# genetics-statistics/GEMMA

Measured on AMD Instinct MI355X. Metric: SNPs/s (-lmm 1 Wald) at n=20k on 1/2/4/8 MI355X; U^T x HBM GB/s vs roofline, higher is better.
Workload: dtype f64 (U^T x as int8-digit MFMA products with exact int32 accumulation; every column of U scaled by its exact maximum and rounded to 6 base-256 digits = 2^-48 of that maximum -- fp64 keeps 2^-53 per entry; value_strict / strict_leg (7g6m: U^T x at or below the fp64 GEMM's own error) and fp64_gemm_path

## Files before the change

gemma_amd/build.py:

```python
import os
import shutil
import subprocess

HERE = os.path.dirname(os.path.abspath(__file__))
CSRC = os.path.join(HERE, "csrc")
LIB = os.path.join(HERE, "libgemma_hip.so")
UNITS = {
    "gemma_hip.hip": ["dgemm_mfma.hip.h", "lmm_grid.hip.h", "i8gemm.hip.h", "i8gemm_sparse.hip.h", "i8gemm_sparse2.hip.h", "i8gemm_sparse2_r16.hip.h", "i8gemm_dense16.hip.h", "lmm_assoc.hip.h",
                      "lmm_search.hip.h", "comm.hip.h", "comm_shm.hpp", "kin_i8.hip.h", "ingest.hip.h", "qc.hip.h", "lm_assoc.hip.h", "mvlmm.hip.h",
                      "mvlmm_kernels.hip.h", "eigh_tu.h", "tu_common.h",
                      "abi_kinship.inc.h", "abi_eigen_qc.inc.h", "abi_lmm_stage.inc.h", "abi_utx.inc.h", "abi_lmm_batch.inc.h",
                      "abi_mvlmm.inc.h", "abi_gxe_lm.inc.h", "abi_kept_comm.inc.h", "abi_vc.inc.h", "vc_tu.h", "abi_prdt.inc.h", "prdt_tu.h",
                      "abi_mqs.inc.h", "mqs_tu.h"],
    "eigh_tu.hip": ["dgemm_mfma.hip.h", "eigh.hip.h", "eigh2.hip.h", "eigh_tu.h", "tu_common.h"],
    "vc_tu.hip": ["dgemm_mfma.hip.h", "spd_inv.hip.h", "vc.hip.h", "vc_tu.h", "tu_common.h", "host_linalg.h", "../../include/gemma_vc_hybrid.hpp"],
    "prdt_tu.hip": ["dgemm_mfma.hip.h", "geno_mv.hip.h", "dev_common.hip.h", "eigh_tu.h", "prdt_tu.h", "tu_common.h"],
    "mqs_tu.hip": ["dgemm_mfma.hip.h", "mqs.hip.h", "dev_common.hip.h", "mqs_tu.h", "tu_common.h", "host_linalg.h"],
    "mvlmm_kernels.hip": ["mvlmm.hip.h", "mvlmm_kernels.hip.h"],
    "mvlmm_kernels_wide.hip": ["mvlmm.hip.h", "mvlmm_kernels.hip.h"],
    "mvlmm_kernels_rt.hip": ["mvlmm.hip.h", "mvlmm_kernels.hip.h"],
    "mvlmm_kernels_d6.hip": ["mvlmm.hip.h", "mvlmm_kernels.hip.h"],
    "mvlmm_kernels_d7.hip": ["mvlmm.hip.h", "mvlmm_kernels.hip.h"],
    "mvlmm_kernels_d8.hip": ["mvlmm.hip.h", "mvlmm_kernels.hip.h"],
}
PUBLIC_HEADER_USERS = ("gemma_hip.hip", "eigh_tu.hip", "vc_tu.hip", "prdt_tu.hip", "mqs_tu.hip")
SOURCES = list(UNITS)
HEADERS = sorted({h for hs in UNITS.values() for h in hs})


def hipcc():
    for cand in (os.environ.get("HIPCC"), "/opt/rocm/bin/hipcc", shutil.which("hipcc")):
        if cand and os.path.exists(cand):
            return cand
    raise RuntimeError("hipcc not found: the gfx950 library cannot be built")


def stale():
    if not os.path.exists(LIB):
        return True
    t = os.path.getmtime(LIB)
    deps = [os.path.join(CSRC, f) for f in SOURCES + HEADERS]
# ... 37 lines not shown
```

gemma_amd/csrc/abi_utx.inc.h:

```cpp

struct I8Dims {
  size_t n, ldk, npad, lpad, mrows;
  int fuse, digits, nplanes;
  int mdrop;
  int complete;
  int epi;
};
static const int *i8_anymiss(const I8Dims &d) { return d.complete ? g_ctx.i8_rowsur.as<int>() + d.lpad : nullptr; }
static int i8_sparse_mode() { return g_ctx.knobs.i8_sparse; }
static int i8_begin(size_t l, I8Dims *d, hipStream_t s, bool allow_epi = true) {
  int rc = i8_prepare_u(s);
  if (rc) return rc;
  d->n = g_ctx.cfg.n; d->ldk = g_ctx.i8_ldk; d->npad = g_ctx.i8_npad;
  d->lpad = round_up(l, i8_sparse_mode() == 2 ? (size_t)S2_BM : (size_t)I8P_BM); d->mrows = 2 * d->lpad;
  d->fuse = (g_ctx.knobs.i8_fuse && (double)d->n * 2.0 * 128.0 * 257.0 < 2147483648.0) ? 1 : 0;
  d->digits = g_ctx.i8_digits;
  d->nplanes = d->fuse ? (d->digits + 1) / 2 : d->digits;
  d->mdrop = (g_ctx.knobs.i8_mdrop && d->fuse && d->digits == 7 && i8_sparse_mode() == 2 && g_ctx.knobs.i8_rows == 16) ? 1 : 0;
  d->complete = (g_ctx.knobs.i8_complete && i8_sparse_mode() == 2 && g_ctx.knobs.i8_rows == 16) ? 1 : 0;
  d->epi = (allow_epi && g_ctx.knobs.i8_epilogue && i8_sparse_mode() == 2 && g_ctx.knobs.i8_rows == 16 && d->nplanes >= 2) ? 1 : 0;
  const size_t c_elems = (size_t)(d->nplanes - d->epi) * d->mrows * d->npad;
  if (g_ctx.i8_A.reserve(d->lpad * d->ldk) || g_ctx.i8_C.reserve(c_elems * 4) || g_ctx.i8_mean.reserve(l * 8))
    return fail(GEMMA_HIP_ENOMEM, "lmm_batch: int8 product buffers (%zu bytes)", d->lpad * d->ldk + c_elems * 4);
  if (d->lpad != l) HIPCHK(hipMemsetAsync(g_ctx.i8_A.p, 0, d->lpad * d->ldk, s));
  return GEMMA_HIP_OK;
}

static int i8_meta_build(const I8Dims &d, hipStream_t s) {
  const int mode = i8_sparse_mode();
  if (mode == 0) return GEMMA_HIP_OK;
  ProfScope ps(GEMMA_STAGE_INGEST, s);
  const size_t nk = d.ldk / I8_BK, total = d.lpad * nk * (mode == 2 ? 4 : 2);
  if (g_ctx.i8_meta.reserve(total * sizeof(uint4)) || g_ctx.i8_rowsur.reserve((d.lpad + 1) * sizeof(int)))
    return fail(GEMMA_HIP_ENOMEM, "lmm_batch: mask words of the sparse product");
  HIPCHK(hipMemsetAsync(g_ctx.i8_rowsur.p, 0, (d.lpad + 1) * sizeof(int), s));
  if (mode == 2)
    hipLaunchKernelGGL(sparse2_meta_kernel, dim3((unsigned)((total + 255) / 256)), dim3(256), 0, s, g_ctx.i8_A.as<int8_t>(),
                       (long)d.lpad, (long)d.ldk, g_ctx.i8_meta.as<uint4>(), g_ctx.i8_rowsur.as<int>(),
                       const_cast<int *>(i8_anymiss(d)));
  else
    hipLaunchKernelGGL(sparse_meta_kernel, dim3((unsigned)((total + 255) / 256)), dim3(256), 0, s, g_ctx.i8_A.as<int8_t>(),
                       (long)d.lpad, (long)d.ldk, g_ctx.i8_meta.as<uint4>(), g_ctx.i8_rowsur.as<int>());
  HIPCHK(hipGetLastError());
  g_ctx.i8_flag_at = (mode == 2 && d.complete) ? (long)d.lpad : -1;
  g_ctx.i8_rowsur_n = (long)d.lpad;
  return GEMMA_HIP_OK;
}

static int raster_for(int tiles_m, int tiles_n, int rb, hipStream_t s, const int2 **map_d) {
  Ctx::RasterSlot *lru = &g_ctx.i8_raster[0];
  for (auto &r : g_ctx.i8_raster) {
    if (r.tm == tiles_m && r.tn == tiles_n && r.rb == rb && r.dev.p) {
      r.used = ++g_ctx.i8_raster_clock;
      *map_d = r.dev.as<int2>();
      return GEMMA_HIP_OK;
    }
    if (r.used < lru->used) lru = &r;
// ... 21 lines not shown
  ProfScope ps(GEMMA_STAGE_UTX_GEMM, s);
  static bool attr_set = false;
  if (!attr_set) {
    HIPCHK(hipFuncSetAttribute(reinterpret_cast<const void *>(i8gemm_packed_kernel_t<true>),
                               hipFuncAttributeMaxDynamicSharedMemorySize, 3 * I8P_STAGE));
    attr_set = true;
  }
  I8PackArgs g;
  g.A = g_ctx.i8_A.as<int8_t>();
  g.Bt = g_ctx.i8_Bt.as<int8_t>();
  g.C = g_ctx.i8_C.as<int>();
  g.ldk = (long)d.ldk; g.ldc = (long)d.npad;
  g.strideB = (long)(d.npad * d.ldk); g.strideC = (long)(d.mrows * d.npad);
  g.m_row0 = (long)d.lpad;
  g.tiles_m = (int)(d.lpad / I8P_BM); g.tiles_n = (int)(d.npad / I8_BN);
  g.nk = (int)(d.ldk / I8_BK);
  g.gm = g_ctx.knobs.i8_gm;
  g.fuse = d.fuse;
  g.digits = d.digits;
  const dim3 grid((unsigned)(g.tiles_m * g.tiles_n), (unsigned)d.nplanes);
  if (mode == 2) {
    static bool attr3 = false;
    if (!attr3) {
      HIPCHK(hipFuncSetAttribute(reinterpret_cast<const void *>(i8gemm_sparse2_kernel),
                                 hipFuncAttributeMaxDynamicSharedMemorySize, S2_NST * S2_STAGE));
      HIPCHK(hipFuncSetAttribute(reinterpret_cast<const void *>(i8gemm_sparse2_r16_kernel),
                                 hipFuncAttributeMaxDynamicSharedMemorySize, S2_R16_LDS));
      HIPCHK(hipFuncSetAttribute(reinterpret_cast<const void *>(i8gemm_sparse2_r16_g_kernel),
                                 hipFuncAttributeMaxDynamicSharedMemorySize, S2_R16_LDS));
      HIPCHK(hipFuncSetAttribute(reinterpret_cast<const void *>(i8gemm_sparse2_r16_ep_kernel),
                                 hipFuncAttributeMaxDynamicSharedMemorySize, S2_R16_LDS));
      HIPCHK(hipFuncSetAttribute(reinterpret_cast<const void *>(i8gemm_sparse2_r16_ep_g_kernel),
                                 hipFuncAttributeMaxDynamicSharedMemorySize, S2_R16_LDS));
      attr3 = true;
    }
    Sparse2Args g2;
    g2.AM = g_ctx.i8_meta.as<uint4>() + (row0 / S2_BM) * (size_t)g.nk * S2_BM * 4;
    g2.Bt = g.Bt; g2.C = g.C + row0 * (size_t)g.ldc - (d.epi ? g.strideC : 0); g2.ldk = g.ldk; g2.ldc = g.ldc; g2.strideB = g.strideB; g2.strideC = g.strideC;
    g2.m_row0 = g.m_row0;
    g2.tiles_m = (int)(rows_pad / S2_BM); g2.tiles_n = (int)(d.npad / S2_BN);
    g2.nk = g.nk; g2.gm = g.gm; g2.fuse = g.fuse; g2.digits = g.digits;
    int raster_rb = 0;
    {
      const int rb = g_ctx.knobs.i8_raster;
      if (rb > 0) {
        const int2 *map_d = nullptr;
        int rc_map = raster_for(g2.tiles_m, g2.tiles_n, rb, s, &map_d);
        if (rc_map) return rc_map;
        g2.tile_map = map_d;
        raster_rb = rb;
      }
    }
    note_utx_kernel(g_ctx.knobs.i8_rows == 32 ? GEMMA_UTX_KERNEL_RECORDS_R32 : GEMMA_UTX_KERNEL_RECORDS_R16, d.digits, d.fuse,
                    raster_rb);
    if (g_ctx.knobs.i8_rows == 32) {
      hipLaunchKernelGGL(i8gemm_sparse2_kernel, dim3((unsigned)(g2.tiles_m * g2.tiles_n), (unsigned)d.nplanes), dim3(512),
                         S2_NST * S2_STAGE, s, g2);
    } else if (d.epi) {
      const unsigned wgs = (unsigned)(g2.tiles_m * g2.tiles_n);
      g2.anymiss = i8_anymiss(d);
      g2.plane0 = 1;
      g2.run_if = g2.anymiss ? 1 : 0;
      hipLaunchKernelGGL(i8gemm_sparse2_r16_kernel, dim3(wgs, (unsigned)d.nplanes - 1u), dim3(512), S2_R16_LDS, s, g2);
      if (g2.anymiss) {
        g2.run_if = 2;
        hipLaunchKernelGGL(i8gemm_sparse2_r16_g_kernel, dim3(wgs, (unsigned)d.nplanes - 1u), dim3(512), S2_R16_LDS, s, g2);
      }
      g2.plane0 = 0;
      g2.UtX = UtX + row0 * ldx; g2.ldx = (long)ldx; g2.l = (long)rows; g2.n = (long)d.n;
      g2.mean = g_ctx.i8_mean.as<double>() + row0; g2.qinv = g_ctx.i8_qinv.as<double>();
      g2.m_scale = 1.0; g2.nplanes = d.nplanes;
      if (d.mdrop) {
        g2.run_if = 0;
        hipLaunchKernelGGL(i8gemm_sparse2_r16_ep_g_kernel, dim3(wgs, 1u), dim3(512), S2_R16_LDS, s, g2);
      } else {
        g2.run_if = g2.anymiss ? 1 : 0;
        hipLaunchKernelGGL(i8gemm_sparse2_r16_ep_kernel, dim3(wgs, 1u), dim3(512), S2_R16_LDS, s, g2);
        if (g2.anymiss) {
          g2.run_if = 2;
          hipLaunchKernelGGL(i8gemm_sparse2_r16_ep_g_kernel, dim3(wgs, 1u), dim3(512), S2_R16_LDS, s, g2);
        }
      }
    } else {
      const unsigned wgs = (unsigned)(g2.tiles_m * g2.tiles_n), first = d.mdrop ? 1u : 0u;
      g2.anymiss = i8_anymiss(d);
      g2.plane0 = (int)first;
      g2.run_if = g2.anymiss ? 1 : 0;
      hipLaunchKernelGGL(i8gemm_sparse2_r16_kernel, dim3(wgs, (unsigned)d.nplanes - first), dim3(512), S2_R16_LDS, s, g2);
      if (g2.anymiss) {
        g2.run_if = 2;
        hipLaunchKernelGGL(i8gemm_sparse2_r16_g_kernel, dim3(wgs, (unsigned)d.nplanes - first), dim3(512), S2_R16_LDS, s, g2);
      }
      if (d.mdrop) {
        g2.plane0 = 0; g2.run_if = 0;
        hipLaunchKernelGGL(i8gemm_sparse2_r16_g_kernel, dim3(wgs, 1u), dim3(512), S2_R16_LDS, s, g2);
      }
    }
  } else if (sparse) {
    static bool attr2 = false;
    if (!attr2) {
      HIPCHK(hipFuncSetAttribute(reinterpret_cast<const void *>(i8gemm_sparse_kernel),
                                 hipFuncAttributeMaxDynamicSharedMemorySize, 3 * SP_STAGE));
      attr2 = true;
    }
    SparseMeta sm;
    sm.m4 = g_ctx.i8_meta.as<uint4>();
    sm.row_surplus = g_ctx.i8_rowsur.as<int>();
    sm.ntiles = (long)g.nk;
    note_utx_kernel(GEMMA_UTX_KERNEL_SPARSE_BYTES, d.digits, d.fuse, 0);
    hipLaunchKernelGGL(i8gemm_sparse_kernel, grid, dim3(512), 3 * SP_STAGE, s, g, sm);
  } else {
    note_utx_kernel(GEMMA_UTX_KERNEL_DENSE_I8, d.digits, d.fuse, 0);
    hipLaunchKernelGGL(i8gemm_packed_kernel_t<true>, grid, dim3(512), 3 * I8P_STAGE, s, g);
// ... 185 lines not shown
```

gemma_amd/csrc/gemma_hip.hip:

```cpp
#include <hip/hip_runtime.h>

#include <cmath>
#include <cstdarg>
#include <cstdio>
#include <cstdlib>
#include <cstring>
#include <string>
#include <vector>

#include "../../include/gemma_hip.h"
#include "tu_common.h"
#include "dgemm_mfma.hip.h"
#include "eigh_tu.h"
#include "vc_tu.h"
#include "prdt_tu.h"
#include "mqs_tu.h"
#include "ingest.hip.h"
#include "lm_assoc.hip.h"
#include "lmm_assoc.hip.h"
#include "lmm_grid.hip.h"
#include "i8gemm.hip.h"
#include "i8gemm_sparse.hip.h"
#include "i8gemm_sparse2.hip.h"
#include "i8gemm_sparse2_r16.hip.h"
#include "i8gemm_dense16.hip.h"
#include "qc.hip.h"
#include "mvlmm.hip.h"
#include "comm.hip.h"
#include "kin_i8.hip.h"

using namespace gemma_hip;

namespace {

struct StageProf {
  std::vector<std::pair<hipEvent_t, hipEvent_t>> ev;
  double acc_ms = 0.0;
  long launches = 0;
};

struct Knobs {
  int utx_i8 = 1;
  int i8_digits = 0;
  int i8_sparse = 2;
  int i8_fuse = 1;
  int i8_gm = 0;
  int i8_raster = S2_DEFAULT_RASTER;
  int i8_rows = 16;
  int i8_scale_max = 1;
  int i8_mdrop = 0;
  int i8_complete = 1;
  int i8_epilogue = 1;
  int dosage_i8 = 1;
  int dosage_rows = 16;
  int overlap = 0;
  int overlap_chunks = 4;
  int table_v2 = 1;
  int table_pf = 0;
  int force_generic = 0;
  int assoc_variant = 44;
  int mvlmm_rt = 0;
  int pipe_cus = 64;
  int kin_i8 = 1, kin_upper = 1, kin_lists = 1, kin_lists_oom = 0;
  long long kin_list_cap = 0;
  static int geti(const char *name, int dflt) {
    const char *e = getenv(name);
    return (e && *e) ? atoi(e) : dflt;
  }
  void load() {
    utx_i8 = geti("GEMMA_HIP_UTX_I8", 1);
    const int dg = geti("GEMMA_HIP_I8_DIGITS", 0);
    i8_digits = (dg == 6 || dg == 7) ? dg : 0;
    const char *es = getenv("GEMMA_HIP_I8_SPARSE");
    i8_sparse = (es && es[0] >= '0' && es[0] <= '2') ? es[0] - '0' : 2;
    const char *ef = getenv("GEMMA_HIP_I8_FUSE");
    i8_fuse = (ef && ef[0] == '0') ? 0 : 1;
    i8_gm = geti("GEMMA_HIP_I8_GM", 0);
    i8_raster = geti("GEMMA_HIP_I8_RASTER", S2_DEFAULT_RASTER);
    i8_rows = geti("GEMMA_HIP_I8_ROWS", 16) == 32 ? 32 : 16;
    const char *esc = getenv("GEMMA_HIP_I8_SCALE");
    i8_scale_max = (esc && strcmp(esc, "pow2") == 0) ? 0 : 1;
    const char *efm = getenv("GEMMA_HIP_I8_FORM");
    i8_mdrop = (efm && strcmp(efm, "7g6m") == 0) ? 1 : 0;
    if (i8_mdrop) i8_digits = 7;
    const char *ecp = getenv("GEMMA_HIP_I8_COMPLETE");
    i8_complete = (ecp && ecp[0] == '0') ? 0 : 1;
    const char *eep = getenv("GEMMA_HIP_I8_EPILOGUE");
    i8_epilogue = (eep && eep[0] == '0') ? 0 : 1;
    const char *ed = getenv("GEMMA_HIP_UTX_DOSAGE_I8");
    dosage_i8 = (ed && ed[0] == '0') ? 0 : 1;
    dosage_rows = geti("GEMMA_HIP_DOSAGE_ROWS", 16) == 32 ? 32 : 16;
    const char *eo = getenv("GEMMA_HIP_OVERLAP");
    overlap = (eo && eo[0] == '1') ? 1 : 0;
    overlap_chunks = geti("GEMMA_HIP_OVERLAP_CHUNKS", 4);
    const char *et = getenv("GEMMA_HIP_TABLE_V2");
    table_v2 = (et && et[0] == '0') ? 0 : 1;
    const char *ep = getenv("GEMMA_HIP_TABLE_PF");
    table_pf = (ep && ep[0] == '1') ? 1 : 0;
    const char *eg = getenv("GEMMA_HIP_FORCE_GENERIC");
    force_generic = (eg && eg[0] == '1') ? 1 : 0;
    assoc_variant = geti("GEMMA_HIP_ASSOC_VARIANT", 44);
    const char *er = getenv("GEMMA_HIP_MVLMM_RT");
    mvlmm_rt = (er && er[0] == '1') ? 1 : 0;
    pipe_cus = geti("GEMMA_HIP_PIPE_CUS", 64);
    const char *k1 = getenv("GEMMA_HIP_KIN_I8"), *k2 = getenv("GEMMA_HIP_KIN_UPPER"), *k3 = getenv("GEMMA_HIP_KIN_LISTS");
    const char *k4 = getenv("GEMMA_HIP_KIN_LISTS_OOM"), *k5 = getenv("GEMMA_HIP_KIN_LIST_CAP");
    kin_i8 = (k1 && k1[0] == '0') ? 0 : 1;
    kin_upper = (k2 && k2[0] == '0') ? 0 : 1;
    kin_lists = (k3 && k3[0] == '0') ? 0 : 1;
    kin_lists_oom = (k4 && k4[0] == '1') ? 1 : 0;
    kin_list_cap = (k5 && *k5) ? atoll(k5) : 0;
  }
};

struct Ctx {
  bool inited = false;
  Knobs knobs;
  int device = -1;
  int verbose = 0;
  std::string last_error;
  hipDeviceProp_t prop;
// ... 374 lines not shown
```

gemma_amd/csrc/i8gemm_sparse2.hip.h:

```cpp
#pragma once
#include <algorithm>
#include <vector>
#include "i8gemm_sparse.hip.h"

namespace gemma_hip {

constexpr int S2_BM = 256, S2_BN = 128;
constexpr int S2_AMB = 16384;
constexpr int S2_STAGE = 32768;
constexpr int S2_NST = 4;
#ifndef S2_ADVANCE
#define S2_ADVANCE 1
#endif
#ifndef S2_LOOPDMA
#define S2_LOOPDMA 1
#endif

struct Sparse2Args {
  const uint4 *AM;
  const int8_t *Bt;
  int *C;
  long ldk, ldc, strideB, strideC, m_row0;
  int tiles_m, tiles_n, nk, gm, fuse, digits;
  int plane0 = 0;
  const int2 *tile_map = nullptr;
  const int *anymiss = nullptr;
  int run_if = 0;
  double *UtX = nullptr;
  long ldx = 0, l = 0, n = 0;
  const double *mean = nullptr, *qinv = nullptr;
  double m_scale = 1.0;
  int nplanes = 0;
};

__global__ __launch_bounds__(256) void sparse2_meta_kernel(const int8_t *__restrict__ A, long lpad, long ldk,
                                                           uint4 *__restrict__ AM, int *__restrict__ row_surplus,
                                                           int *anymiss = nullptr ) {
  const long nk = ldk / I8_BK;
  const long id = (long)blockIdx.x * 256 + threadIdx.x;
  if (id >= lpad * nk * 4) return;
  const int c = (int)(id & 3);
  const long rr = (id >> 2) & 255, tk = id >> 10;
  const long tmi = tk / nk, kt = tk - tmi * nk;
  const long row = tmi * S2_BM + rr;
  const int p = c >> 1, h = c & 1;
  const int8_t *base = A + row * ldk + kt * I8_BK;
  unsigned w[4];
#pragma unroll
  for (int e = 0; e < 2; ++e) {
    const int8_t *src = base + 32 * (2 * p + e) + 16 * h;
    unsigned g2 = 0;
#pragma unroll
    for (int i = 0; i < 4; ++i) g2 |= (*reinterpret_cast<const unsigned *>(src + 4 * i) & 0x03030303u) << (2 * i);
    w[e] = g2;
  }
  {
    const int8_t *src = base + 32 * (2 * p + h);
    unsigned idx = 0, bits = 0;
    int surplus = 0;
    for (int gq = 0; gq < 8; ++gq) {
      const unsigned word = *reinterpret_cast<const unsigned *>(src + 4 * gq);
      const unsigned m = (word >> 4) & 0x01010101u;
      const unsigned pat = (m | (m >> 7) | (m >> 14) | (m >> 21)) & 0xFu;
      const int cnt = __popc(pat);
      const int p0 = cnt >= 1 ? __ffs(pat) - 1 : 0;
// ... 325 lines not shown
```

gemma_amd/csrc/i8gemm_sparse2_r16.hip.h:

```cpp
#pragma once
#include "i8gemm_sparse2.hip.h"

#ifndef S2_R16_PREP_SPREAD
#define S2_R16_PREP_SPREAD 0
#endif
#ifndef S2_R16_NST
#define S2_R16_NST 4
#endif
#ifndef S2_R16_ABL_NO_S
#define S2_R16_ABL_NO_S 0
#endif
#ifndef S2_R16_ABL_NO_D
#define S2_R16_ABL_NO_D 0
#endif

namespace gemma_hip {

constexpr int S2_R16_LDS = S2_R16_NST * S2_STAGE;

template <bool WITH_S, bool COMBINE = false>
__device__ __forceinline__ void s2_r16_body(const Sparse2Args &g) {
  extern __shared__ __attribute__((aligned(1024))) int8_t i8lds[];
  constexpr bool NO_S = !WITH_S || S2_R16_ABL_NO_S;
  if (g.run_if) {
    const int any = __builtin_amdgcn_readfirstlane(*g.anymiss);
    if ((g.run_if == 1) != (any != 0)) return;
  }
  int tm, tn;
  if (g.tile_map) {
    const int2 t2 = g.tile_map[blockIdx.x];
    tm = __builtin_amdgcn_readfirstlane(t2.x);
    tn = __builtin_amdgcn_readfirstlane(t2.y);
  } else {
    const int nwg = gridDim.x, b = blockIdx.x;
    const int q_ = nwg >> 3, r = nwg & 7, x = b & 7, o = b >> 3;
    const int L = (x < r ? x * (q_ + 1) : r * (q_ + 1) + (x - r) * q_) + o;
    const int GM = g.gm > 0 ? g.gm : 8;
    const int per_group = GM * g.tiles_n;
    const int grp = L / per_group;
    const int first_m = grp * GM;
    const int gsz = min(g.tiles_m - first_m, GM);
    const int in = L - grp * per_group;
    tm = first_m + in % gsz;
    tn = in / gsz;
  }
  const int plane = blockIdx.y + g.plane0;
  const int odd = g.digits & 1;
  const int d_first = g.fuse ? (odd ? (plane == 0 ? 0 : 2 * plane) : 2 * plane + 1) : plane;
  const int nd = (g.fuse && !(odd && plane == 0)) ? 2 : 1;
  const int t = threadIdx.x, lane = t & 63;
  const int wave = __builtin_amdgcn_readfirstlane(t >> 6);
  const int r16 = lane & 15, q = lane >> 4;

  const uint4 *asrc[2];
  const int8_t *bsrc[2];
  int adst[2], bdst[2];
// ... 54 lines not shown
    ga[i][1] = s2_unpack_g((q >> 1) ? rec[i][1][1] : rec[i][1][0]);                                               \
    ix[i] = (q >> 1) ? rec[i][1][2] : rec[i][0][2];                                                               \
    ms[i] = s2_expand((q >> 1) ? rec[i][1][3] : rec[i][0][3]);                                                    \
    asm volatile("" ::"v"(rec[i][0]), "v"(rec[i][1]));                                                            \
  } while (0)
#define GS_PREP_G(i, P) ga[i][P] = s2_unpack_g((q >> 1) ? rec[i][P][1] : rec[i][P][0])
#define GS_PREP_M(i)                                                                                              \
  do {                                                                                                            \
    ix[i] = (q >> 1) ? rec[i][1][2] : rec[i][0][2];                                                               \
    ms[i] = s2_expand((q >> 1) ? rec[i][1][3] : rec[i][0][3]);                                                    \
    asm volatile("" ::"v"(rec[i][0]), "v"(rec[i][1]));                                                            \
  } while (0)
#define GS_D(i, SB, P, SL)                                                                                        \
  do {                                                                                                            \
    if (!S2_R16_ABL_NO_D)                                                                                         \
      asm volatile("s_nop 1\n\tv_mfma_i32_16x16x64_i8 %0, %1, %2, %0"                                             \
                   : "+v"(accg[i][SB])                                                                            \
                   : "v"(ga[i][P]), "v"(__builtin_shufflevector(T[SL], T[SL], 4 * (P), 4 * (P) + 1, 4 * (P) + 2, 4 * (P) + 3))); \
  } while (0)
#define GS_S(i, SB, SL)                                                                                           \
  do {                                                                                                            \
    if (!NO_S)                                                                                                    \
      asm volatile("s_nop 1\n\tv_smfmac_i32_16x16x128_i8 %0, %1, %2, %3" : "+v"(accm[i][SB]) : "v"(ms[i]), "v"(T[SL]), "v"(ix[i])); \
  } while (0)
#define GS_STEP(SB, SL, X)                                                                                        \
  do {                                                                                                            \
    GS_D(0, SB, 0, SL); GEMMA_SB();                                                                               \
    GS_D(1, SB, 0, SL); X; GEMMA_SB();                                                                            \
    GS_D(0, SB, 1, SL); GEMMA_SB();                                                                               \
    GS_D(1, SB, 1, SL); GEMMA_SB();                                                                               \
    GS_S(0, SB, SL); GEMMA_SB();                                                                                  \
    GS_S(1, SB, SL); GEMMA_SB();                                                                                  \
  } while (0)
#define GS_KTILE(SC, SN, SD, MORE, LOAD3, VMW)                                                                    \
  do {                                                                                                            \
    GS_STEP(0, 0, { GS_RT(SC, 3, 3); if (LOAD3) GS_DMA_A(0, SD); });                                               \
    GS_STEP(1, 1, { GS_RT(SC, 4, 0); if (LOAD3) GS_DMA_A(1, SD); });                                               \
    GS_STEP(2, 2, { GS_RT(SC, 5, 1); if (LOAD3) GS_DMA_B(0, SD); });                                               \
    GS_STEP(3, 3, { GS_RT(SC, 6, 2); if (LOAD3) GS_DMA_B(1, SD); });                                               \
    GS_STEP(4, 0, { GS_RT(SC, 7, 3); });                                                                           \
    asm volatile("s_waitcnt vmcnt(" #VMW ")" ::: "memory");                                                       \
    __builtin_amdgcn_s_barrier();                                                                                 \
    GEMMA_SB();                                                                                                   \
    GS_STEP(5, 1, { if (MORE) { GS_RREC(SN, 0, 0); GS_RREC(SN, 0, 1); GS_RREC(SN, 1, 0); GS_RREC(SN, 1, 1);       \
                                GS_RT(SN, 0, 0); } });                                                             \
    GS_STEP(6, 2, { if (MORE) { GS_RT(SN, 1, 1); } });                                                             \
    if (S2_R16_PREP_SPREAD && (MORE)) {                                                                           \
      GS_D(0, 7, 0, 3); GEMMA_SB();                                                                               \
      GS_D(1, 7, 0, 3); { GS_RT(SN, 2, 2); GS_PREP_G(0, 0); } GEMMA_SB();                                          \
      GS_D(0, 7, 1, 3); { GS_PREP_G(1, 0); } GEMMA_SB();                                                           \
      GS_D(1, 7, 1, 3); { GS_PREP_G(0, 1); } GEMMA_SB();                                                           \
      GS_S(0, 7, 3); { GS_PREP_G(1, 1); } GEMMA_SB();                                                              \
      GS_S(1, 7, 3); { GS_PREP_M(0); } GEMMA_SB();                                                                 \
      { GS_PREP_M(1); } GEMMA_SB();                                                                                \
    } else {                                                                                                      \
      GS_STEP(7, 3, { if (MORE) { GS_RT(SN, 2, 2); } });                                                           \
      if (MORE) { GS_PREP(0); GS_PREP(1); }                                                                       \
      GEMMA_SB();                                                                                                 \
    }                                                                                                             \
  } while (0)

  if (wave >= 4) __builtin_amdgcn_s_setprio(1);
  const int nk = g.nk;
  for (int dd = 0; dd < nd; ++dd) {
    if (dd > 0) {
      asm volatile("s_nop 15\n\ts_nop 7" ::: "memory");
#pragma unroll
      for (int i = 0; i < 2; ++i)
#pragma unroll
        for (int j = 0; j < 8; ++j)
#pragma unroll
          for (int r = 0; r < 4; ++r) {
            accg[i][j][r] <<= 8;
            if (WITH_S) accm[i][j][r] <<= 8;
          }
    }
    GS_INIT_SRC(d_first - dd);
#pragma unroll
    for (int j = 0; j < 2; ++j) { GS_DMA_A(j, 0); GS_DMA_B(j, 0); }
    if (nk > 1) {
#pragma unroll
      for (int j = 0; j < 2; ++j) { GS_DMA_A(j, S2_STAGE); GS_DMA_B(j, S2_STAGE); }
    }
    if (nk > 2) {
#pragma unroll
      for (int j = 0; j < 2; ++j) { GS_DMA_A(j, 2 * S2_STAGE); GS_DMA_B(j, 2 * S2_STAGE); }
    }
    if (S2_R16_NST == 5 && nk > 3) {
#pragma unroll
      for (int j = 0; j < 2; ++j) { GS_DMA_A(j, 3 * S2_STAGE); GS_DMA_B(j, 3 * S2_STAGE); }
      asm volatile("s_waitcnt vmcnt(12)" ::: "memory");
    } else if (nk > 2) {
      asm volatile("s_waitcnt vmcnt(8)" ::: "memory");
    } else if (nk > 1) {
      asm volatile("s_waitcnt vmcnt(4)" ::: "memory");
    } else {
      asm volatile("s_waitcnt vmcnt(0)" ::: "memory");
    }
    __builtin_amdgcn_s_barrier();
    GEMMA_SB();
    GS_RT(0, 0, 0);
    GS_RT(0, 1, 1);
    GS_RT(0, 2, 2);
    GS_RREC(0, 0, 0); GS_RREC(0, 0, 1); GS_RREC(0, 1, 0); GS_RREC(0, 1, 1);
    GS_PREP(0);
    GS_PREP(1);
    GEMMA_SB();

    int sc = 0, sn = S2_STAGE, s2 = 2 * S2_STAGE, s3 = 3 * S2_STAGE, sd = (S2_R16_NST - 1) * S2_STAGE;
#define GS_ROTATE()                                                                                               \
  do {                                                                                                            \
    const int tmp = sc;                                                                                           \
    sc = sn; sn = s2;                                                                                             \
    if (S2_R16_NST == 5) { s2 = s3; s3 = sd; } else { s2 = sd; }                                                  \
    sd = tmp;                                                                                                     \
  } while (0)
    int kt = 0;
    if (S2_R16_NST == 5) {
      for (; kt + 4 < nk; ++kt) {
        GS_KTILE(sc, sn, sd, true, true, 12);
        GS_ROTATE();
      }
      if (nk >= 4) {
        GS_KTILE(sc, sn, sd, true, false, 8);
        GS_ROTATE();
      }
    } else {
      for (; kt + 3 < nk; ++kt) {
        GS_KTILE(sc, sn, sd, true, true, 8);
        GS_ROTATE();
      }
    }
    if (nk >= 3) {
      GS_KTILE(sc, sn, sd, true, false, 4);
      GS_ROTATE();
    }
    if (nk >= 2) {
      GS_KTILE(sc, sn, sd, true, false, 0);
      GS_ROTATE();
    }
    GS_KTILE(sc, sn, sd, false, false, 0);
#undef GS_ROTATE
  }

  asm volatile("s_nop 15\n\ts_nop 7" ::: "memory");
  if constexpr (COMBINE) {
    const int np = g.nplanes;
    const bool load_m = !(g.anymiss && __builtin_amdgcn_readfirstlane(*g.anymiss) == 0);
    const double w_hi = g.fuse ? 65536.0 : 256.0;
    const double w0 = (g.fuse && !odd) ? 65536.0 : 256.0;
    const long row_w = (long)tm * S2_BM + wave * 32, col_w = (long)tn * S2_BN;
    const long row_l = row_w + 4 * q, col_l = col_w + r16;
    const unsigned lo_c = (unsigned)((4 * q * g.ldc + r16) * 4), lo_x = (unsigned)((4 * q * g.ldx + r16) * 8);
#define EP_AT(T, BASE, LO) (*(T *)((const char *)(BASE) + (LO)))
#define EP_LOAD(DG, DM, I, H, P)                                                                                  \
  do {                                                                                                            \
    const int *cp_ = g.C + (long)(P) * g.strideC + (row_w + 16 * (I)) * g.ldc + col_w + 32 * (H);                 \
    _Pragma("unroll") for (int k_ = 0; k_ < 2; ++k_) _Pragma("unroll") for (int r_ = 0; r_ < 4; ++r_) {           \
      DG[4 * k_ + r_] = EP_AT(const int, cp_ + r_ * g.ldc + 16 * k_, lo_c);                                       \
      DM[4 * k_ + r_] = load_m ? EP_AT(const int, cp_ + (g.m_row0 + r_) * g.ldc + 16 * k_, lo_c) : 0;             \
    }                                                                                                             \
  } while (0)
    int cg[8], cm[8];
#pragma unroll
    for (int e = 0; e < 8; ++e) cg[e] = cm[e] = 0;
    if (np > 1) EP_LOAD(cg, cm, 0, 0, np - 1);
#pragma unroll
    for (int b = 0; b < 8; ++b) {
      const int i = b >> 2, h = b & 3;
      double tg[8], tk[8];
#pragma unroll
      for (int e = 0; e < 8; ++e) tg[e] = tk[e] = 0.0;
      for (int p = np - 1; p >= 1; --p) {
        int ng[8], nm[8];
#pragma unroll
        for (int e = 0; e < 8; ++e) ng[e] = nm[e] = 0;
        if (p > 1) EP_LOAD(ng, nm, i, h, p - 1);
        else if (b < 7) EP_LOAD(ng, nm, (b + 1) >> 2, (b + 1) & 3, np - 1);
#pragma unroll
// ... 19 lines not shown
                fma(ms, tk[e], tg[e]) * EP_AT(const double, g.qinv + col_w + 16 * sb, (unsigned)(8 * r16));
        }
      }
    }
#undef EP_AT
#undef EP_LOAD
  } else {
    int *Cg = g.C + (long)plane * g.strideC;
#pragma unroll
    for (int i = 0; i < 2; ++i)
#pragma unroll
      for (int sb = 0; sb < 8; ++sb) {
        const long col = (long)tn * S2_BN + 16 * sb + r16;
#pragma unroll
        for (int r = 0; r < 4; ++r) {
          const long row = (long)tm * S2_BM + wave * 32 + 16 * i + 4 * q + r;
          Cg[row * g.ldc + col] = accg[i][sb][r];
          if (WITH_S) Cg[(g.m_row0 + row) * g.ldc + col] = accm[i][sb][r];
        }
      }
  }
#undef GS_INIT_SRC
#undef GS_DMA_A
#undef GS_DMA_B
#undef GS_RREC
#undef GS_RT
#undef GS_PREP
#undef GS_PREP_G
#undef GS_PREP_M
#undef GS_D
#undef GS_S
#undef GS_STEP
#undef GS_KTILE
}

__global__ __launch_bounds__(512, 2) void i8gemm_sparse2_r16_kernel(Sparse2Args g) { s2_r16_body<true>(g); }
__global__ __launch_bounds__(512, 2) void i8gemm_sparse2_r16_g_kernel(Sparse2Args g) { s2_r16_body<false>(g); }
__global__ __launch_bounds__(512, 2) void i8gemm_sparse2_r16_ep_kernel(Sparse2Args g) { s2_r16_body<true, true>(g); }
__global__ __launch_bounds__(512, 2) void i8gemm_sparse2_r16_ep_g_kernel(Sparse2Args g) { s2_r16_body<false, true>(g); }

}
```

Baseline: 362,500.

## Store int8 digit-plane partials in a fragment-ordered image and stream them via LDS

Adds a new plane-image layout: the upper-plane GEMM kernels write each wave's accumulator fragments contiguously instead of as a row-major C matrix. The combine epilogue kernel prefetches those fragments with global_load_lds into a per-wave LDS ring, starting during its last k-tile, and recombines the digits from LDS. This is enabled by default through i8_epilogue=2 when the fused path has four or fewer planes. The aim is fully coalesced partial-product traffic and overlap of those loads with the final MFMA work. The cost is a larger LDS footprint and new indexing that must match exactly between producer and consumer; the pad memset is also narrowed to the padding rows only.

```diff
diff --git a/gemma_amd/build.py b/gemma_amd/build.py
--- a/gemma_amd/build.py
+++ b/gemma_amd/build.py
@@ -6,7 +6,7 @@
 CSRC = os.path.join(HERE, "csrc")
 LIB = os.path.join(HERE, "libgemma_hip.so")
 UNITS = {
-    "gemma_hip.hip": ["dgemm_mfma.hip.h", "lmm_grid.hip.h", "i8gemm.hip.h", "i8gemm_sparse.hip.h", "i8gemm_sparse2.hip.h", "i8gemm_sparse2_r16.hip.h", "i8gemm_dense16.hip.h", "lmm_assoc.hip.h",
+    "gemma_hip.hip": ["dgemm_mfma.hip.h", "lmm_grid.hip.h", "i8gemm.hip.h", "i8gemm_sparse.hip.h", "i8gemm_sparse2.hip.h", "i8gemm_sparse2_r16.hip.h", "plane_image.h", "i8gemm_dense16.hip.h", "lmm_assoc.hip.h",
                       "lmm_search.hip.h", "comm.hip.h", "comm_shm.hpp", "kin_i8.hip.h", "ingest.hip.h", "qc.hip.h", "lm_assoc.hip.h", "mvlmm.hip.h",
                       "mvlmm_kernels.hip.h", "eigh_tu.h", "tu_common.h",
                       "abi_kinship.inc.h", "abi_eigen_qc.inc.h", "abi_lmm_stage.inc.h", "abi_utx.inc.h", "abi_lmm_batch.inc.h",
diff --git a/gemma_amd/csrc/abi_utx.inc.h b/gemma_amd/csrc/abi_utx.inc.h
--- a/gemma_amd/csrc/abi_utx.inc.h
+++ b/gemma_amd/csrc/abi_utx.inc.h
@@ -19,10 +19,11 @@
   d->mdrop = (g_ctx.knobs.i8_mdrop && d->fuse && d->digits == 7 && i8_sparse_mode() == 2 && g_ctx.knobs.i8_rows == 16) ? 1 : 0;
   d->complete = (g_ctx.knobs.i8_complete && i8_sparse_mode() == 2 && g_ctx.knobs.i8_rows == 16) ? 1 : 0;
   d->epi = (allow_epi && g_ctx.knobs.i8_epilogue && i8_sparse_mode() == 2 && g_ctx.knobs.i8_rows == 16 && d->nplanes >= 2) ? 1 : 0;
-  const size_t c_elems = (size_t)(d->nplanes - d->epi) * d->mrows * d->npad;
+  if (d->epi && g_ctx.knobs.i8_epilogue == 2 && d->fuse && d->nplanes <= 4) d->epi = 2;
+  const size_t c_elems = (size_t)(d->nplanes - (d->epi ? 1 : 0)) * d->mrows * d->npad;
   if (g_ctx.i8_A.reserve(d->lpad * d->ldk) || g_ctx.i8_C.reserve(c_elems * 4) || g_ctx.i8_mean.reserve(l * 8))
     return fail(GEMMA_HIP_ENOMEM, "lmm_batch: int8 product buffers (%zu bytes)", d->lpad * d->ldk + c_elems * 4);
-  if (d->lpad != l) HIPCHK(hipMemsetAsync(g_ctx.i8_A.p, 0, d->lpad * d->ldk, s));
+  if (d->lpad != l) HIPCHK(hipMemsetAsync(g_ctx.i8_A.as<int8_t>() + l * d->ldk, 0, (d->lpad - l) * d->ldk, s));
   return GEMMA_HIP_OK;
 }
 
@@ -110,13 +111,22 @@
                                  hipFuncAttributeMaxDynamicSharedMemorySize, S2_R16_LDS));
       HIPCHK(hipFuncSetAttribute(reinterpret_cast<const void *>(i8gemm_sparse2_r16_ep_g_kernel),
                                  hipFuncAttributeMaxDynamicSharedMemorySize, S2_R16_LDS));
+      HIPCHK(hipFuncSetAttribute(reinterpret_cast<const void *>(i8gemm_sparse2_r16_img_kernel),
+                                 hipFuncAttributeMaxDynamicSharedMemorySize, S2_R16_LDS));
+      HIPCHK(hipFuncSetAttribute(reinterpret_cast<const void *>(i8gemm_sparse2_r16_img_g_kernel),
+                                 hipFuncAttributeMaxDynamicSharedMemorySize, S2_R16_LDS));
+      HIPCHK(hipFuncSetAttribute(reinterpret_cast<const void *>(i8gemm_sparse2_r16_ep2_kernel),
+                                 hipFuncAttributeMaxDynamicSharedMemorySize, S2_R16_EP2_LDS));
+      HIPCHK(hipFuncSetAttribute(reinterpret_cast<const void *>(i8gemm_sparse2_r16_ep2_g_kernel),
+                                 hipFuncAttributeMaxDynamicSharedMemorySize, S2_R16_EP2_LDS));
       attr3 = true;
     }
     Sparse2Args g2;
     g2.AM = g_ctx.i8_meta.as<uint4>() + (row0 / S2_BM) * (size_t)g.nk * S2_BM * 4;
-    g2.Bt = g.Bt; g2.C = g.C + row0 * (size_t)g.ldc - (d.epi ? g.strideC : 0); g2.ldk = g.ldk; g2.ldc = g.ldc; g2.strideB = g.strideB; g2.strideC = g.strideC;
+    g2.Bt = g.Bt; g2.C = d.epi == 2 ? g.C : g.C + row0 * (size_t)g.ldc - (d.epi ? g.strideC : 0); g2.ldk = g.ldk; g2.ldc = g.ldc; g2.strideB = g.strideB; g2.strideC = g.strideC;
     g2.m_row0 = g.m_row0;
-    g2.tiles_m = (int)(rows_pad / S2_BM); g2.tiles_n = (int)(d.npad / S2_BN);
+    g2.tiles_m = (int)(rows_pad / S2_BM); g2.tiles_n = (int)((d.n + S2_BN - 1) / S2_BN);
+    g2.img_tm0 = (int)(row0 / S2_BM); g2.nplanes = d.nplanes;
     g2.nk = g.nk; g2.gm = g.gm; g2.fuse = g.fuse; g2.digits = g.digits;
     int raster_rb = 0;
     {
@@ -139,24 +149,29 @@
       g2.anymiss = i8_anymiss(d);
       g2.plane0 = 1;
       g2.run_if = g2.anymiss ? 1 : 0;
-      hipLaunchKernelGGL(i8gemm_sparse2_r16_kernel, dim3(wgs, (unsigned)d.nplanes - 1u), dim3(512), S2_R16_LDS, s, g2);
+      const bool img = d.epi == 2;
+      const dim3 upper(wgs, (unsigned)d.nplanes - 1u);
+      hipLaunchKernelGGL(img ? i8gemm_sparse2_r16_img_kernel : i8gemm_sparse2_r16_kernel, upper, dim3(512), S2_R16_LDS, s, g2);
       if (g2.anymiss) {
         g2.run_if = 2;
-        hipLaunchKernelGGL(i8gemm_sparse2_r16_g_kernel, dim3(wgs, (unsigned)d.nplanes - 1u), dim3(512), S2_R16_LDS, s, g2);
+        hipLaunchKernelGGL(img ? i8gemm_sparse2_r16_img_g_kernel : i8gemm_sparse2_r16_g_kernel, upper, dim3(512), S2_R16_LDS, s, g2);
       }
       g2.plane0 = 0;
       g2.UtX = UtX + row0 * ldx; g2.ldx = (long)ldx; g2.l = (long)rows; g2.n = (long)d.n;
       g2.mean = g_ctx.i8_mean.as<double>() + row0; g2.qinv = g_ctx.i8_qinv.as<double>();
-      g2.m_scale = 1.0; g2.nplanes = d.nplanes;
+      g2.m_scale = 1.0;
+      const auto ep = img ? i8gemm_sparse2_r16_ep2_kernel : i8gemm_sparse2_r16_ep_kernel;
+      const auto ep_g = img ? i8gemm_sparse2_r16_ep2_g_kernel : i8gemm_sparse2_r16_ep_g_kernel;
+      const unsigned ep_lds = img ? S2_R16_EP2_LDS : S2_R16_LDS;
       if (d.mdrop) {
         g2.run_if = 0;
-        hipLaunchKernelGGL(i8gemm_sparse2_r16_ep_g_kernel, dim3(wgs, 1u), dim3(512), S2_R16_LDS, s, g2);
+        hipLaunchKernelGGL(ep_g, dim3(wgs, 1u), dim3(512), ep_lds, s, g2);
       } else {
         g2.run_if = g2.anymiss ? 1 : 0;
-        hipLaunchKernelGGL(i8gemm_sparse2_r16_ep_kernel, dim3(wgs, 1u), dim3(512), S2_R16_LDS, s, g2);
+        hipLaunchKernelGGL(ep, dim3(wgs, 1u), dim3(512), ep_lds, s, g2);
         if (g2.anymiss) {
           g2.run_if = 2;
-          hipLaunchKernelGGL(i8gemm_sparse2_r16_ep_g_kernel, dim3(wgs, 1u), dim3(512), S2_R16_LDS, s, g2);
+          hipLaunchKernelGGL(ep_g, dim3(wgs, 1u), dim3(512), ep_lds, s, g2);
         }
       }
     } else {
diff --git a/gemma_amd/csrc/gemma_hip.hip b/gemma_amd/csrc/gemma_hip.hip
--- a/gemma_amd/csrc/gemma_hip.hip
+++ b/gemma_amd/csrc/gemma_hip.hip
@@ -50,7 +50,7 @@
   int i8_scale_max = 1;
   int i8_mdrop = 0;
   int i8_complete = 1;
-  int i8_epilogue = 1;
+  int i8_epilogue = 2;
   int dosage_i8 = 1;
   int dosage_rows = 16;
   int overlap = 0;
@@ -86,7 +86,7 @@
     const char *ecp = getenv("GEMMA_HIP_I8_COMPLETE");
     i8_complete = (ecp && ecp[0] == '0') ? 0 : 1;
     const char *eep = getenv("GEMMA_HIP_I8_EPILOGUE");
-    i8_epilogue = (eep && eep[0] == '0') ? 0 : 1;
+    i8_epilogue = (eep && eep[0] == '0') ? 0 : (eep && eep[0] == '1') ? 1 : 2;
     const char *ed = getenv("GEMMA_HIP_UTX_DOSAGE_I8");
     dosage_i8 = (ed && ed[0] == '0') ? 0 : 1;
     dosage_rows = geti("GEMMA_HIP_DOSAGE_ROWS", 16) == 32 ? 32 : 16;
diff --git a/gemma_amd/csrc/i8gemm_sparse2.hip.h b/gemma_amd/csrc/i8gemm_sparse2.hip.h
--- a/gemma_amd/csrc/i8gemm_sparse2.hip.h
+++ b/gemma_amd/csrc/i8gemm_sparse2.hip.h
@@ -31,6 +31,7 @@
   const double *mean = nullptr, *qinv = nullptr;
   double m_scale = 1.0;
   int nplanes = 0;
+  int img_tm0 = 0;
 };
 
 __global__ __launch_bounds__(256) void sparse2_meta_kernel(const int8_t *__restrict__ A, long lpad, long ldk,
diff --git a/gemma_amd/csrc/i8gemm_sparse2_r16.hip.h b/gemma_amd/csrc/i8gemm_sparse2_r16.hip.h
--- a/gemma_amd/csrc/i8gemm_sparse2_r16.hip.h
+++ b/gemma_amd/csrc/i8gemm_sparse2_r16.hip.h
@@ -1,5 +1,6 @@
 #pragma once
 #include "i8gemm_sparse2.hip.h"
+#include "plane_image.h"
 
 #ifndef S2_R16_PREP_SPREAD
 #define S2_R16_PREP_SPREAD 0
@@ -17,11 +18,27 @@
 namespace gemma_hip {
 
 constexpr int S2_R16_LDS = S2_R16_NST * S2_STAGE;
-
-template <bool WITH_S, bool COMBINE = false>
+constexpr int S2_EP2_RING = S2_R16_LDS / 8;
+constexpr int S2_EP2_AUX = 1024 + 256;
+constexpr int S2_R16_EP2_LDS = S2_R16_LDS + 8 * S2_EP2_AUX;
+static_assert(S2_EP2_RING == 16384 && S2_R16_EP2_LDS <= 160 * 1024, "the plane ring is sized for four 32-KiB stages");
+
+__device__ __forceinline__ void s2_ep2_wait_vm(int n) {
+  switch (n) {
+#define S2_EP2_W(N) case N: asm volatile("s_waitcnt vmcnt(" #N ")" ::: "memory"); break;
+    S2_EP2_W(12) S2_EP2_W(11) S2_EP2_W(10) S2_EP2_W(9) S2_EP2_W(8) S2_EP2_W(7) S2_EP2_W(6) S2_EP2_W(5) S2_EP2_W(4) S2_EP2_W(3)
+    S2_EP2_W(2) S2_EP2_W(1)
+#undef S2_EP2_W
+    default: asm volatile("s_waitcnt vmcnt(0)" ::: "memory"); break;
+  }
+}
+
+template <bool WITH_S, bool COMBINE = false, bool IMAGE = false>
 __device__ __forceinline__ void s2_r16_body(const Sparse2Args &g) {
   extern __shared__ __attribute__((aligned(1024))) int8_t i8lds[];
   constexpr bool NO_S = !WITH_S || S2_R16_ABL_NO_S;
+  bool load_m = true;
+  if constexpr (COMBINE && IMAGE) load_m = !(g.anymiss && __builtin_amdgcn_readfirstlane(*g.anymiss) == 0);
   if (g.run_if) {
     const int any = __builtin_amdgcn_readfirstlane(*g.anymiss);
     if ((g.run_if == 1) != (any != 0)) return;
@@ -142,7 +159,7 @@
     GS_S(0, SB, SL); GEMMA_SB();                                                                                  \
     GS_S(1, SB, SL); GEMMA_SB();                                                                                  \
   } while (0)
-#define GS_KTILE(SC, SN, SD, MORE, LOAD3, VMW)                                                                    \
+#define GS_KTILE(SC, SN, SD, MORE, LOAD3, VMW, PF)                                                                  \
   do {                                                                                                            \
     GS_STEP(0, 0, { GS_RT(SC, 3, 3); if (LOAD3) GS_DMA_A(0, SD); });                                               \
     GS_STEP(1, 1, { GS_RT(SC, 4, 0); if (LOAD3) GS_DMA_A(1, SD); });                                               \
@@ -154,7 +171,7 @@
     GEMMA_SB();                                                                                                   \
     GS_STEP(5, 1, { if (MORE) { GS_RREC(SN, 0, 0); GS_RREC(SN, 0, 1); GS_RREC(SN, 1, 0); GS_RREC(SN, 1, 1);       \
                                 GS_RT(SN, 0, 0); } });                                                             \
-    GS_STEP(6, 2, { if (MORE) { GS_RT(SN, 1, 1); } });                                                             \
+    GS_STEP(6, 2, { if (MORE) { GS_RT(SN, 1, 1); } PF; });                                                         \
     if (S2_R16_PREP_SPREAD && (MORE)) {                                                                           \
       GS_D(0, 7, 0, 3); GEMMA_SB();                                                                               \
       GS_D(1, 7, 0, 3); { GS_RT(SN, 2, 2); GS_PREP_G(0, 0); } GEMMA_SB();                                          \
@@ -170,6 +187,49 @@
     }                                                                                                             \
   } while (0)
 
+#define EP2_GEOMETRY(LANE)                                                                                        \
+  const int np = g.nplanes;  \
+  const int npl = np - 1;                                                                                         \
+  const int pq = npl * (load_m ? 2 : 1);                                                                          \
+  const int depth = pq > 4 ? 2 : 4;                                                                               \
+  const char *img_l = reinterpret_cast<const char *>(g.C + plane_image_piece((long)(g.img_tm0 + tm) * g.tiles_n + tn, wave, 0, np, 1, 0) + \
+                                                     plane_image_in_piece(LANE, 0));                              \
+  const long quad_b = plane_image_quad_dwords(np) * 4;                                                            \
+  int8_t *ring = i8lds + wave * S2_EP2_RING;                                                                      \
+  int8_t *aux = i8lds + S2_R16_LDS + wave * S2_EP2_AUX
+#define EP2_ISSUE(QD)                                                                                             \
+  do {                                                                                                            \
+    const char *s_ = img_l + (QD) * quad_b;                                                                       \
+    int8_t *d_ = ring + ((QD) & (depth - 1)) * (pq * 1024);                                                       \
+    for (int p_ = npl; p_ >= 1; --p_) {                                                                           \
+      __builtin_amdgcn_global_load_lds((gemma_gptr_t)(s_ + (p_ - 1) * 2048), (gemma_lptr_t)d_, 16, 0, 0);         \
+      d_ += 1024;                                                                                                 \
+      if (load_m) {                                                                                               \
+        __builtin_amdgcn_global_load_lds((gemma_gptr_t)(s_ + (p_ - 1) * 2048 + 1024), (gemma_lptr_t)d_, 16, 0, 0); \
+        d_ += 1024;                                                                                               \
+      }                                                                                                           \
+    }                                                                                                             \
+  } while (0)
+#define EP2_PROLOGUE()                                                                                            \
+  do {                                                                                                            \
+    int ln_ = lane;  \
+    asm volatile("" : "+v"(ln_));                                                                                 \
+    EP2_GEOMETRY(ln_);                                                                                            \
+    _Pragma("unroll") for (int j_ = 0; j_ < 4; ++j_) {                                                            \
+      long c_ = (long)tn * S2_BN + 32 * j_ + (ln_ >> 1);                                                          \
+      c_ = c_ < g.n ? c_ : g.n - 1;                                                                               \
+      __builtin_amdgcn_global_load_lds((gemma_gptr_t)(reinterpret_cast<const char *>(g.qinv + c_) + 4 * (ln_ & 1)), \
+                                       (gemma_lptr_t)(aux + 256 * j_), 4, 0, 0);                                  \
+    }                                                                                                             \
+    {                                                                                                             \
+      long r_ = (long)tm * S2_BM + wave * 32 + (ln_ >> 1);                                                        \
+      r_ = r_ < g.l ? r_ : g.l - 1;                                                                               \
+      __builtin_amdgcn_global_load_lds((gemma_gptr_t)(reinterpret_cast<const char *>(g.mean + r_) + 4 * (ln_ & 1)), \
+                                       (gemma_lptr_t)(aux + 1024), 4, 0, 0);                                      \
+    }                                                                                                             \
+    for (int qd_ = 0; qd_ < depth; ++qd_) EP2_ISSUE(qd_);                                                         \
+  } while (0)
+
   if (wave >= 4) __builtin_amdgcn_s_setprio(1);
   const int nk = g.nk;
   for (int dd = 0; dd < nd; ++dd) {
@@ -228,33 +288,92 @@
     int kt = 0;
     if (S2_R16_NST == 5) {
       for (; kt + 4 < nk; ++kt) {
-        GS_KTILE(sc, sn, sd, true, true, 12);
+        GS_KTILE(sc, sn, sd, true, true, 12, );
         GS_ROTATE();
       }
       if (nk >= 4) {
-        GS_KTILE(sc, sn, sd, true, false, 8);
+        GS_KTILE(sc, sn, sd, true, false, 8, );
         GS_ROTATE();
       }
     } else {
       for (; kt + 3 < nk; ++kt) {
-        GS_KTILE(sc, sn, sd, true, true, 8);
+        GS_KTILE(sc, sn, sd, true, true, 8, );
         GS_ROTATE();
       }
     }
     if (nk >= 3) {
-      GS_KTILE(sc, sn, sd, true, false, 4);
+      GS_KTILE(sc, sn, sd, true, false, 4, );
       GS_ROTATE();
     }
     if (nk >= 2) {
-      GS_KTILE(sc, sn, sd, true, false, 0);
+      GS_KTILE(sc, sn, sd, true, false, 0, );
       GS_ROTATE();
     }
-    GS_KTILE(sc, sn, sd, false, false, 0);
+    GS_KTILE(sc, sn, sd, false, false, 0, { if constexpr (COMBINE && IMAGE) { if (dd == nd - 1) { EP2_PROLOGUE(); } } });
 #undef GS_ROTATE
   }
 
   asm volatile("s_nop 15\n\ts_nop 7" ::: "memory");
-  if constexpr (COMBINE) {
+  if constexpr (COMBINE && IMAGE) {
+    EP2_GEOMETRY(lane);
+    const double w_hi = g.fuse ? 65536.0 : 256.0;
+    const double w0 = (g.fuse && !odd) ? 65536.0 : 256.0;
+    const long row_l = (long)tm * S2_BM + plane_image_row(wave, 0, lane, 0), col_l = (long)tn * S2_BN + plane_image_col(0, lane);
+    const double *qv_l = reinterpret_cast<const double *>(aux) + r16, *mean_l = reinterpret_cast<const double *>(aux + 1024) + 4 * q;
+    double res[16][4];
+#define EP2_QUAD(QD)                                                                                              \
+  do {                                                                                                            \
+    constexpr int i = (QD) >> 3, sb = (QD) & 7;                                                                   \
+    s2_ep2_wait_vm(min(depth - 1, 15 - (QD)) * pq);                    \
+    const int8_t *sl = ring + ((QD) & (depth - 1)) * (pq * 1024) + lane * 16;                                     \
+    double tg[4] = {0.0, 0.0, 0.0, 0.0}, tk[4] = {0.0, 0.0, 0.0, 0.0};                                            \
+    for (int p = npl; p >= 1; --p) {                                                                              \
+      const i32x4 cg = *reinterpret_cast<const i32x4 *>(sl);                                                      \
+      sl += 1024;                                                                                                 \
+      i32x4 cm = (i32x4){0, 0, 0, 0};                                                                             \
+      if (load_m) {                                                                                               \
+        cm = *reinterpret_cast<const i32x4 *>(sl);                                                                \
+        sl += 1024;                                                                                               \
+      }                                                                                                           \
+      _Pragma("unroll") for (int r = 0; r < 4; ++r) {                                                             \
+        tg[r] = tg[r] * w_hi + (double)cg[r];                                                                     \
+        tk[r] = tk[r] * w_hi + (double)cm[r];                                                                     \
+      }                                                                                                           \
+    }                                                                                                             \
+    asm volatile("s_waitcnt lgkmcnt(0)" ::: "memory");  \
+    if ((QD) + depth < 16) EP2_ISSUE((QD) + depth);                                                               \
+    const double qv = qv_l[16 * sb];                                                                              \
+    _Pragma("unroll") for (int r = 0; r < 4; ++r) {                                                               \
+      const bool row_in = row_l + 16 * i + r < g.l;                                                               \
+      const double ms = row_in ? mean_l[16 * i + r] * g.m_scale : 0.0;                                            \
+      const int m0 = WITH_S ? accm[i][sb][r] : 0;                                                                 \
+      tg[r] = tg[r] * w0 + (double)accg[i][sb][r];                                                                \
+      tk[r] = tk[r] * w0 + (double)m0;                                                                            \
+      res[QD][r] = fma(ms, tk[r], tg[r]) * qv;                                                                    \
+      asm volatile("" : "+v"(res[QD][r]));  \
+    }                                                                                                             \
+  } while (0)
+#define EP2_STORE(QD)                                                                                             \
+  do {                                                                                                            \
+    constexpr int i = (QD) >> 3, sb = (QD) & 7;                                                                   \
+    _Pragma("unroll") for (int r = 0; r < 4; ++r)                                                                 \
+      if (row_l + 16 * i + r < g.l && col_l + 16 * sb < g.n) g.UtX[(row_l + 16 * i + r) * g.ldx + col_l + 16 * sb] = res[QD][r]; \
+  } while (0)
+    EP2_QUAD(0); EP2_QUAD(1); EP2_QUAD(2); EP2_QUAD(3); EP2_QUAD(4); EP2_QUAD(5); EP2_QUAD(6); EP2_QUAD(7);
+    EP2_QUAD(8); EP2_QUAD(9); EP2_QUAD(10); EP2_QUAD(11); EP2_QUAD(12); EP2_QUAD(13); EP2_QUAD(14); EP2_QUAD(15);
+    EP2_STORE(0); EP2_STORE(1); EP2_STORE(2); EP2_STORE(3); EP2_STORE(4); EP2_STORE(5); EP2_STORE(6); EP2_STORE(7);
+    EP2_STORE(8); EP2_STORE(9); EP2_STORE(10); EP2_STORE(11); EP2_STORE(12); EP2_STORE(13); EP2_STORE(14); EP2_STORE(15);
+#undef EP2_QUAD
+#undef EP2_STORE
+  } else if constexpr (IMAGE) {
+    int *ip = g.C + plane_image_piece((long)(g.img_tm0 + tm) * g.tiles_n + tn, wave, 0, g.nplanes, plane, 0) + plane_image_in_piece(lane, 0);
+    const long quad_d = plane_image_quad_dwords(g.nplanes);
+#pragma unroll
+    for (int qd = 0; qd < 16; ++qd) {
+      *reinterpret_cast<i32x4 *>(ip + qd * quad_d) = accg[qd >> 3][qd & 7];
+      if (WITH_S) *reinterpret_cast<i32x4 *>(ip + qd * quad_d + PI_PIECE) = accm[qd >> 3][qd & 7];
+    }
+  } else if constexpr (COMBINE) {
     const int np = g.nplanes;
     const bool load_m = !(g.anymiss && __builtin_amdgcn_readfirstlane(*g.anymiss) == 0);
     const double w_hi = g.fuse ? 65536.0 : 256.0;
@@ -340,11 +459,18 @@
 #undef GS_S
 #undef GS_STEP
 #undef GS_KTILE
+#undef EP2_GEOMETRY
+#undef EP2_ISSUE
+#undef EP2_PROLOGUE
 }
 
 __global__ __launch_bounds__(512, 2) void i8gemm_sparse2_r16_kernel(Sparse2Args g) { s2_r16_body<true>(g); }
 __global__ __launch_bounds__(512, 2) void i8gemm_sparse2_r16_g_kernel(Sparse2Args g) { s2_r16_body<false>(g); }
 __global__ __launch_bounds__(512, 2) void i8gemm_sparse2_r16_ep_kernel(Sparse2Args g) { s2_r16_body<true, true>(g); }
 __global__ __launch_bounds__(512, 2) void i8gemm_sparse2_r16_ep_g_kernel(Sparse2Args g) { s2_r16_body<false, true>(g); }
+__global__ __launch_bounds__(512, 2) void i8gemm_sparse2_r16_img_kernel(Sparse2Args g) { s2_r16_body<true, false, true>(g); }
+__global__ __launch_bounds__(512, 2) void i8gemm_sparse2_r16_img_g_kernel(Sparse2Args g) { s2_r16_body<false, false, true>(g); }
+__global__ __launch_bounds__(512, 2) void i8gemm_sparse2_r16_ep2_kernel(Sparse2Args g) { s2_r16_body<true, true, true>(g); }
+__global__ __launch_bounds__(512, 2) void i8gemm_sparse2_r16_ep2_g_kernel(Sparse2Args g) { s2_r16_body<false, true, true>(g); }
 
 }
diff --git a/gemma_amd/csrc/plane_image.h b/gemma_amd/csrc/plane_image.h
--- /dev/null
+++ b/gemma_amd/csrc/plane_image.h
@@ -0,0 +1,26 @@
+#pragma once
+
+#if defined(__HIPCC__)
+#define GEMMA_PI_FN __host__ __device__ __forceinline__
+#else
+#define GEMMA_PI_FN inline
+#endif
+
+namespace gemma_hip {
+
+constexpr int PI_WAVES = 8;
+constexpr int PI_QUADS = 16;
+constexpr int PI_LANES = 64;
+constexpr int PI_PIECE = 256;
+constexpr int PI_TILE_M = 256, PI_TILE_N = 128;
+
+GEMMA_PI_FN long plane_image_piece(long tile, int wave, int quad, int np, int plane, int gm) {
+  return ((((tile * PI_WAVES + wave) * PI_QUADS + quad) * (long)(np - 1) + (plane - 1)) * 2 + gm) * PI_PIECE;
+}
+GEMMA_PI_FN int plane_image_in_piece(int lane, int r) { return lane * 4 + r; }
+GEMMA_PI_FN long plane_image_quad_dwords(int np) { return (long)(np - 1) * 2 * PI_PIECE; }
+GEMMA_PI_FN long plane_image_tile_dwords(int np) { return plane_image_quad_dwords(np) * PI_QUADS * PI_WAVES; }
+GEMMA_PI_FN int plane_image_row(int wave, int quad, int lane, int r) { return wave * 32 + 16 * (quad >> 3) + 4 * (lane >> 4) + r; }
+GEMMA_PI_FN int plane_image_col(int quad, int lane) { return 16 * (quad & 7) + (lane & 15); }
+
+}
```

After: 365,000 (median of 6 runs). No clear change (+0.7%).
